# leslie-wang/hevcbitstream

Measured on AMD Instinct MI355X. Metric: Annex-B GB/s scanned + NAL units/s, 16 GiB synthetic stream, 1/2/4/8 MI355X, higher is better.
Workload: dtype u8

## Files before the change

hevcbitstream_amd/csrc/hbs_common.h:

```cpp
#ifndef HBS_COMMON_H
#define HBS_COMMON_H

#include <stdint.h>
#include <stddef.h>
#include "../../include/hevcbitstream_amd.h"

#if defined(__HIPCC__) && !defined(HBS_HOST_SIM)
#define HBS_HD __host__ __device__ __forceinline__
#define HBS_D  __device__ __forceinline__
#define HBS_M  __host__ __device__ __forceinline__
#else
#define HBS_HD static inline
#define HBS_D  static inline
#define HBS_M  inline
#endif

namespace hbs {

constexpr int kThreads         = 512;
constexpr int kWaves           = kThreads / 64;
constexpr int kBlockBytes      = 64;
constexpr int kBlocksPerThread = 2;
constexpr int kThreadBytes     = kBlockBytes * kBlocksPerThread;
constexpr int kTileBytes       = kThreads * kThreadBytes;
// ... 44 lines not shown
static_assert(sizeof(AheadCtl) == 64, "one line");
HBS_HD unsigned long long ahead_stamp_of(unsigned long long call) { return (call + 1ull) << 2; }

struct Carver {
    uint8_t* base;
    uint64_t at;
    template <class T> T* take(uint64_t bytes, uint64_t pack = 256)
    {
        T* const p = base ? reinterpret_cast<T*>(base + at) : nullptr;
        at += (bytes + pack - 1) / pack * pack;
        return p;
    }
};

constexpr uint64_t kOutCapMax = 1ull << 46;

constexpr uint32_t kDenseOneIn = 44;
constexpr int kExactFlagMin = 2;
constexpr uint32_t kDenseOneInIndexOnly = 9;
HBS_HD bool probe_says_dense(uint32_t chunks, uint32_t flagged, uint32_t one_in = kDenseOneIn) { return (uint64_t)flagged * one_in > (uint64_t)chunks; }
constexpr uint32_t kMidTwoIn = 13;
enum : int { kProbeSparse = 0, kProbeMid = 1, kProbeDense = 2 };
HBS_HD int probe_class(uint32_t chunks, uint32_t flagged, bool index_only)
{
    if (!probe_says_dense(chunks, flagged, index_only ? kDenseOneInIndexOnly : kDenseOneIn)) return kProbeSparse;
    return (uint64_t)flagged * kMidTwoIn > 2ull * (uint64_t)chunks ? kProbeDense : kProbeMid;
}
HBS_HD int probe_variant(uint32_t chunks, uint32_t flagged, bool index_only)
{
    const int c = probe_class(chunks, flagged, index_only);
    if (index_only) return c == kProbeSparse ? 5 : 2;
    return c == kProbeSparse ? 4 : c == kProbeMid ? 6 : 2;
}
enum : int { kGateNone = 0, kGateIfSparse = 1, kGateIfDense = 2, kGateIfSparseIdx = 3, kGateIfDenseIdx = 4, kGateIfMid = 5 };
#ifdef __HIPCC__
__device__ __forceinline__ int probe_class_dev(const RunHeader* __restrict__ hdr, bool index_only)
{
    const int lane = threadIdx.x & 63;
    uint32_t c = hdr->probe_slot[lane][0], f = hdr->probe_slot[lane][1];
#pragma unroll
    for (int d = 32; d >= 1; d >>= 1) { c += __shfl_xor(c, d, 64); f += __shfl_xor(f, d, 64); }
    return probe_class(c, f, index_only);
}
__device__ __forceinline__ bool gate_closed(int gate, const RunHeader* __restrict__ hdr)
{
    if (gate == kGateNone) return false;
    const bool idx = gate == kGateIfSparseIdx || gate == kGateIfDenseIdx;
    const int c = probe_class_dev(hdr, idx);
    if (idx) return (gate == kGateIfSparseIdx) != (c == kProbeSparse);
    const int want = gate == kGateIfSparse ? kProbeSparse : gate == kGateIfMid ? kProbeMid : kProbeDense;
    return c != want;
}
template <int kUnused = 0> __global__ void k_clear(uint8_t* __restrict__ p, uint64_t bytes)
{
    const uint64_t tid = (uint64_t)blockIdx.x * blockDim.x + threadIdx.x, step = (uint64_t)gridDim.x * blockDim.x;
    uint64_t head = (16u - (uint32_t)(reinterpret_cast<uintptr_t>(p) & 15u)) & 15u;
    if (head > bytes) head = bytes;
    const uint64_t whole = (bytes - head) / 16u;
    uint4* const q = reinterpret_cast<uint4*>(p + head);
    const uint4 z = make_uint4(0, 0, 0, 0);
    for (uint64_t i = tid; i < whole; i += step) q[i] = z;
    for (uint64_t i = tid; i < head; i += step) p[i] = 0;
    for (uint64_t i = head + 16u * whole + tid; i < bytes; i += step) p[i] = 0;
}
inline hipError_t clear_async(void* p, uint64_t bytes, hipStream_t st)
{
    if (!bytes) return hipSuccess;
    const uint64_t want = (bytes / 16u + 255u) / 256u;
    k_clear<0><<<dim3((unsigned)(want < 1 ? 1 : want > 1024 ? 1024 : want)), dim3(256), 0, st>>>(static_cast<uint8_t*>(p), bytes);
    return hipGetLastError();
}
inline hipError_t begin_launches(hipEvent_t ev_begin, hipStream_t st)
{
    return ev_begin ? hipEventRecord(ev_begin, st) : hipSuccess;
}
inline hipError_t end_launches(hipEvent_t ev_end, hipStream_t st)
{
    const hipError_t e = hipGetLastError();
    return e != hipSuccess || !ev_end ? e : hipEventRecord(ev_end, st);
}
#endif


HBS_HD uint32_t popc64(uint64_t v) { return (uint32_t)__builtin_popcountll(v); }
// ... 35 lines not shown
```

hevcbitstream_amd/csrc/hbs_scan.h:

```cpp
#ifndef HBS_SCAN_H
#define HBS_SCAN_H

#include <hip/hip_runtime_api.h>
#include <cassert>
#include "hbs_common.h"

namespace hbs {

struct ScanArgs {
    const uint8_t* stream;
    uint64_t n;
    hbs_nal_entry* index;
    uint64_t index_cap;
    uint8_t* rbsp;
    uint64_t rbsp_cap;
    unsigned long long* desc;
    RunHeader* hdr;
    uint8_t* tail;
    void* ws5;
    hbs_summary* summary;
    unsigned long long* ahead_cand;
    uint32_t* ahead_list;
    AheadCtl* ahead_ctl;
    void* ahead_tab;
    int grid_blocks;
    int grid_blocks4;
    int grid_blocks4r24;
    int first_static;
    int spare_wgs;
    hipEvent_t ev_begin, ev_end;
    int cus;
    int variant;
};

int scan_grid_blocks(int device, int* blocks_per_cu_out);
hipError_t launch_scan_extract(const ScanArgs& a, hipStream_t st);
inline bool scan_uses_index_only(uint64_t n, int variant, const void* rbsp)
{
    return rbsp == nullptr && (variant == 5 || (variant == 0 && n >= (1ull << 30)));
}
bool scan_takes_small_path(uint64_t n, uint64_t index_cap, int variant);

int scan4_grid_blocks(int device, int* blocks_per_cu_out);
int scan4_tile_bytes();
int scan4_tail_bytes();
void launch_scan_prologue(const ScanArgs& a, uint64_t desc_words, bool probe, int tail_tile_bytes , hipStream_t st);
void scan4_launch_kernel(const ScanArgs& a, uint64_t num_tiles, int gate, hipStream_t st);
int scan4r24_grid_blocks(int device, int* blocks_per_cu_out);
int scan4r24_tile_bytes();
void scan4r24_launch_kernel(const ScanArgs& a, uint64_t num_tiles, int gate, hipStream_t st);
uint64_t scan4_ahead_entry_bytes();
bool scan4_counts_ahead(uint64_t n);
void launch_scan_ahead4(const ScanArgs& a, uint64_t num_tiles, int gate, hipStream_t st);
inline uint64_t lay_scan_ahead(Carver& w, ScanArgs& a, uint64_t tiles)
{
    const uint64_t word = sizeof(unsigned long long), listed = sizeof(uint32_t), entry = scan4_ahead_entry_bytes() - word - listed;
    assert(entry == 64);
    a.ahead_ctl = w.take<AheadCtl>(sizeof(AheadCtl), 1);
    a.ahead_tab = w.take<void>(tiles * entry, 1);
    a.ahead_cand = w.take<unsigned long long>(tiles * word, 1);
    const uint64_t cleared = w.at;
    a.ahead_list = w.take<uint32_t>(tiles * listed, 1);
    return cleared;
}

uint64_t scan5_workspace_bytes(uint64_t stream_bytes);
struct Geo5 { int rows; int strided; uint64_t tiles, grid; };
Geo5 scan5_geometry(uint64_t n, uint64_t waves);
int scan5_tile_rows(uint64_t n, uint64_t waves);
void launch_scan_index5(const ScanArgs& a, int gate, hipStream_t st);

}
#endif
```

hevcbitstream_amd/csrc/hbs_scan.hip:

```cpp
#include <hip/hip_runtime.h>
#include "hbs_tile.h"
#include "hbs_scan.h"

namespace hbs {

#ifdef HBS_PHASE_TIMING
__device__ unsigned long long g_phase_cycles[1024][8];
#define HBS_T_DECL unsigned long long t_prev = __builtin_amdgcn_s_memtime(), t_acc[8] = {0,0,0,0,0,0,0,0};
#define HBS_T_MARK(i) { const unsigned long long t_now = __builtin_amdgcn_s_memtime(); t_acc[i] += t_now - t_prev; t_prev = t_now; }
#define HBS_T_COUNT(i, v) { t_acc[i] += (v); }
#define HBS_T_FLUSH if (threadIdx.x == 0 && blockIdx.x < 1024) { for (int i = 0; i < 8; ++i) g_phase_cycles[blockIdx.x][i] = t_acc[i]; }
__device__ int g_stop_after = 99;
#define HBS_T_STOP(i) if (g_stop_after == (i)) break;
#else
#define HBS_T_STOP(i)
#define HBS_T_DECL
#define HBS_T_MARK(i)
#define HBS_T_COUNT(i, v)
#define HBS_T_FLUSH
#endif

constexpr int kSlowCap = 256;

struct WaveSlot {
// ... 540 lines not shown
    if (per_cu < 1) per_cu = 1;
    if (blocks_per_cu_out) *blocks_per_cu_out = per_cu;
    return prop.multiProcessorCount * per_cu;
}

hipError_t launch_scan_extract(const ScanArgs& a, hipStream_t st)
{
    hipError_t e;
    const bool automatic = a.variant == 0;
    if (scan_takes_small_path(a.n, a.index_cap, a.variant)) {
        if (a.ev_begin) { e = hipEventRecord(a.ev_begin, st); if (e != hipSuccess) return e; }
        k_scan_small<<<1, dim3(kThreads), 0, st>>>(a.stream, a.n, a.index, a.index_cap, a.rbsp, a.rbsp_cap, a.desc, a.hdr, a.summary);
        if (a.ev_end) { e = hipEventRecord(a.ev_end, st); if (e != hipSuccess) return e; }
        return hipGetLastError();
    }
    const bool index_only = scan_uses_index_only(a.n, a.variant, a.rbsp);
    const int sparse_variant = ((a.variant == 5 && !index_only) || automatic) ? 4 : a.variant;
    const uint64_t tiles4 = (a.n + (uint64_t)scan4_tile_bytes() - 1) / (uint64_t)scan4_tile_bytes();
    const uint64_t tiles6 = (a.n + (uint64_t)scan4r24_tile_bytes() - 1) / (uint64_t)scan4r24_tile_bytes();
    const uint64_t tiles2 = (a.n + (uint64_t)kTileBytes - 1) / (uint64_t)kTileBytes;
    const uint64_t num_tiles = automatic ? tiles2 : sparse_variant == 4 ? tiles4 : sparse_variant == 6 ? tiles6 : tiles2;
    const int tail_tile = ((!index_only && sparse_variant == 4) || sparse_variant == 6 || automatic) ? scan4_tile_bytes() : 0;
    launch_scan_prologue(a, num_tiles * 2, automatic && a.n != 0, tail_tile, st);
    hipError_t first = hipSuccess;
    auto note = [&](hipError_t x) { if (first == hipSuccess && x != hipSuccess) first = x; };
    if (num_tiles) {
        uint64_t grid = (uint64_t)a.grid_blocks;
        if (grid > tiles2) grid = tiles2;
        if (a.ev_begin) note(hipEventRecord(a.ev_begin, st));
        if (index_only && !automatic) {
            launch_scan_index5(a, kGateNone, st);
        } else if (!automatic && sparse_variant == 4) {
            launch_scan_ahead4(a, tiles4, kGateNone, st);
            scan4_launch_kernel(a, tiles4, kGateNone, st);
        } else if (!automatic && sparse_variant == 6) {
            scan4r24_launch_kernel(a, tiles6, kGateNone, st);
        } else if (automatic) {
            if (index_only) launch_scan_index5(a, kGateIfSparseIdx, st);
            else { launch_scan_ahead4(a, tiles4, kGateIfSparse, st); scan4_launch_kernel(a, tiles4, kGateIfSparse, st); }
            if (!index_only) scan4r24_launch_kernel(a, tiles6, kGateIfMid, st);
            k_scan_extract<<<dim3((unsigned)grid), dim3(kThreads), 0, st>>>(
                a.stream, a.n, tiles2, a.index, a.index_cap, a.rbsp, a.rbsp_cap, a.desc, a.hdr, index_only ? kGateIfDenseIdx : kGateIfDense);
        } else {
            k_scan_extract<<<dim3((unsigned)grid), dim3(kThreads), 0, st>>>(
                a.stream, a.n, tiles2, a.index, a.index_cap, a.rbsp, a.rbsp_cap, a.desc, a.hdr, kGateNone);
        }
        if (a.ev_end) note(hipEventRecord(a.ev_end, st));
    }
    const uint64_t may = a.index_cap < a.n / 3 + 1 ? a.index_cap : a.n / 3 + 1;
    uint64_t fb = (may + 1023) / 1024;
    fb = fb < (uint64_t)kFinishBlocksMin ? (uint64_t)kFinishBlocksMin : fb > (uint64_t)kFinishBlocksMax ? (uint64_t)kFinishBlocksMax : fb;
    k_scan_finish<<<dim3((unsigned)fb), 256, 0, st>>>(a.stream, a.n, a.index, a.index_cap, a.rbsp, a.rbsp_cap, a.hdr, a.summary, a.ahead_ctl);
    note(hipGetLastError());
    return first;
}

}
```

hevcbitstream_amd/csrc/hbs_scan4.hip:

```cpp
#define HBS4_ROWS 48
#include "hbs_scan4_impl.h"
```

hevcbitstream_amd/csrc/hbs_scan4_impl.h:

```cpp
#include <hip/hip_runtime.h>
#ifndef HBS4_ROWS
#error "compile hbs_scan4.hip / hbs_scan4_r24.hip, which set HBS4_ROWS and include this file"
#endif
#include "hbs_wave.h"
#include "hbs_sparse.h"
#include "hbs_scan.h"
#include "hbs_elems.h"
#if HBS4_ROWS == 48
#include "hbs_scan4_rows48.h"
#define HBS4_KERNEL k_scan_extract4
#elif HBS4_ROWS == 24
#include "hbs_scan4_rows24.h"
#define HBS4_KERNEL k_scan_extract4_r24
#else
#error "no row lists for this HBS4_ROWS: scripts/set_rows4.py"
#endif
#define HBS4_MAIN (HBS4_ROWS == 48)

namespace hbs {
namespace {

#ifdef HBS_PHASE_TIMING
static __device__ unsigned long long g_phase_cycles4[1024][8];
#define HBS4_T_DECL unsigned long long t_prev = __builtin_amdgcn_s_memtime(), t_acc[8] = {0,0,0,0,0,0,0,0};
#define HBS4_T_MARK(i) { const unsigned long long t_now = __builtin_amdgcn_s_memtime(); t_acc[i] += t_now - t_prev; t_prev = t_now; }
#define HBS4_T_COUNT(i, v) { t_acc[i] += (v); }
#define HBS4_T_FLUSH if (threadIdx.x == 0 && blockIdx.x < 1024) { for (int i = 0; i < 8; ++i) g_phase_cycles4[blockIdx.x][i] = t_acc[i]; }
static __device__ uint32_t g_dbg4[4096];
constexpr unsigned kTl4Tiles = 1u << 17;
static __device__ unsigned long long g_tl4[kTl4Tiles][4];
static __device__ unsigned long long g_tlwho4[kTl4Tiles];
#define HBS4_TL(tile, k, bit) { if (threadIdx.x == 0 && (tile) < kTl4Tiles) { g_tl4[tile][k] = (wall_clock64() & ~1ull) | (unsigned long long)(bit); \
    if ((k) == 0) g_tlwho4[tile] = (unsigned long long)blockIdx.x | ((unsigned long long)(__builtin_amdgcn_s_getreg(63508) & 15u) << 28) | \
                                   ((unsigned long long)__builtin_amdgcn_s_getreg(63492) << 32); } }
static __device__ int g_fake_lb4 = 0;
#define HBS4_DBG(code) code
#else
#define HBS4_DBG(code)
#define HBS4_TL(tile, k, bit)
#define HBS4_T_DECL
#define HBS4_T_MARK(i)
#define HBS4_T_COUNT(i, v)
#define HBS4_T_FLUSH
#endif

constexpr int kWgPerCu = 2;
constexpr int kElemWaves = HBS4_ROWS == 48 ? 2 : 4;
constexpr int kCopyDepth = 3;
static_assert(k4Rows == HBS4_ROWS, "hbs_sparse.h takes the geometry from HBS4_ROWS");
constexpr int kParkRows = HBS4_PARK_ROWS;

struct RowRegs {
#define HBS_DECL(r) u32x4 q##r;
    HBS_ROWS(HBS_DECL)
#undef HBS_DECL
    uint32_t before;
    uint32_t before2;
    uint32_t after;
};

constexpr int kDepCap = 64;
constexpr uint32_t kDenseElems = HBS4_ROWS == 48 ? 512 : 1024;

struct Lds4 {
    uint32_t wave_tot[k4Waves];
    uint16_t wlist[k4Waves][kDenseElems];
    uint32_t seg[kDenseElems + 1];
    u32x4 rec[kDenseElems][3];
    Deposit dep[k4Waves][kDepCap];
    u32x4 park[kParkRows ? kElemWaves : 1][kParkRows ? kParkRows : 1][kParkRows ? 64 : 1];
    unsigned long long ex_kept, ex_nals;
    uint32_t ex_inside, ex_ok;
    uint32_t ticket;
    TileAgg wagg[k4Waves];
    TileAgg bagg[kDenseElems / k4ElemPass];
};


constexpr int kDenseAhead = 8;
static_assert(k4Rows % kDenseAhead == 0, "whole batches of rows");
template <class F>
__device__ __forceinline__ void dense_rows(const uint8_t* src, uint64_t wseg, int lane, F&& f)
// ... 171 lines not shown
        HBS4_TL(tile, 2, 0)
        __builtin_amdgcn_s_setprio(0);
        const uint32_t tile_kept = tagg.known + (ex.inside ? tagg.sig : 0u);
        const bool can = rbsp != nullptr && ex.kept + tile_kept <= rbsp_cap;
        if (lane == 0) {
            l.ex_kept = ex.kept; l.ex_nals = ex.nals; l.ex_inside = ex.inside;
            l.ex_ok = !ok ? 0u : (rbsp != nullptr && !can) ? 2u : 1u;
            if (ok && rbsp != nullptr && !can) atomicMax(&hdr->error, (uint32_t)(-HBS_E_CAPACITY));
            if (ok && last_tile) {
                const Prefix incl = fold(ex, tagg);
                hdr->final_kept = incl.kept; hdr->final_nals = incl.nals; hdr->final_inside = incl.inside;
            }
        }
    } else {
        __builtin_amdgcn_s_setprio(0);
    }
    __syncthreads();
    if (l.ex_ok == 0u) return false;
    Prefix excl;
    {
        Prefix ex;
        ex.kept = l.ex_kept; ex.nals = l.ex_nals; ex.inside = l.ex_inside;
        excl = prefix_uniform4(ex);
    }
    dense_emit(src, wseg, n, before, before2, after, chunk0, lane, before_me, excl, rbsp != nullptr && l.ex_ok == 1u, rbsp + excl.kept, tgt,
               &l.dep[wv][lane & (kDepCap - 1)].xpp);
    __syncthreads();
    if (tid == 0) l.ticket = ticket_base + atomicAdd(&hdr->ticket, 1u);
    __syncthreads();
    HBS4_TL(tile, 3, 0)
    return true;
}

}

#if HBS4_MAIN
__global__ __launch_bounds__(k4Threads)
void k_scan_ahead4(const uint8_t* __restrict__ stream, uint64_t n, uint64_t num_tiles, unsigned long long* __restrict__ cand,
                   const uint32_t* __restrict__ list, const AheadCtl* __restrict__ ctl,
                   AheadEntry* __restrict__ tab, const RunHeader* __restrict__ hdr, int gate)
{
    const uint32_t marked = ctl->listed;
    const unsigned long long stamp = ahead_stamp_of(ctl->call);
    if (blockIdx.x >= marked || gate_closed(gate, hdr)) return;
    __shared__ uint32_t rough[k4Waves];
    __shared__ TileAgg wagg[k4Waves];
    const int tid = threadIdx.x, lane = tid & 63;
    const int wv = __builtin_amdgcn_readfirstlane(tid >> 6);
    for (uint32_t i = blockIdx.x; i < marked; i += gridDim.x) {
        const uint64_t tile = list[i];
        if (tile + 1 >= num_tiles) continue;
        const uint64_t base = tile * (uint64_t)k4TileBytes;
        const uint64_t wseg = base + (uint64_t)(wv * k4WaveBytes);
        uint32_t mine = 0;
#pragma unroll 4
        for (int r = 0; r < k4Rows; ++r) {
            const Quad q = *reinterpret_cast<const Quad*>(stream + wseg + (uint64_t)r * k4RowBytes + (uint64_t)lane * 16u);
            mine += (uint32_t)__builtin_popcountll(__ballot(chunk_flag(0xFFFFFFFFu, q.x, q.y, q.z, q.w, 0xFFFFFFFFu)));
        }
        __syncthreads();
        if (lane == 0) rough[wv] = mine;
        __syncthreads();
        const bool walk = rough[0] + rough[1] + rough[2] + rough[3] >= kAheadRoughMin;
        if (!walk) continue;
        const uint32_t before = (wseg >= 4) ? stream_load4(stream + wseg - 4) : 0xFFFFFFFFu;
        const uint32_t before2 = (wseg >= 8) ? stream_load4(stream + wseg - 8) : 0xFFFFFFFFu;
        const uint32_t after = (wv != k4Waves - 1) ? stream_load4(stream + wseg + k4WaveBytes) : load_dword_guarded(stream, (int64_t)(wseg + k4WaveBytes), n);
        const TileAgg wa = dense_aggregate(stream, wseg, n, before, before2, after, (uint32_t)(64 * k4Rows * wv), lane);
        if (lane == 0) wagg[wv] = wa;
        __syncthreads();
        if (tid == 0) {
            AheadEntry e;
#pragma unroll
            for (int w = 0; w < k4Waves; ++w) e.w[w] = wagg[w];
            tab[tile] = e;
            cand[tile] = stamp | kAheadDone;
        }
    }
}

uint64_t scan4_ahead_entry_bytes() { return sizeof(AheadEntry) + sizeof(unsigned long long) + sizeof(uint32_t); }
bool scan4_counts_ahead(uint64_t n) { return n >= kAheadMinBytes; }

void launch_scan_ahead4(const ScanArgs& a, uint64_t num_tiles, int gate, hipStream_t st)
{
    if (!a.ahead_cand || !a.ahead_tab || num_tiles < 2) return;
    k_scan_ahead4<<<dim3(1024), dim3(k4Threads), 0, st>>>(a.stream, a.n, num_tiles, a.ahead_cand, a.ahead_list, a.ahead_ctl,
                                                         static_cast<AheadEntry*>(a.ahead_tab), a.hdr, gate);
}

#endif

__global__ __launch_bounds__(k4Threads, kWgPerCu)
void HBS4_KERNEL(const uint8_t* __restrict__ stream, uint64_t n, uint64_t num_tiles,
                 hbs_nal_entry* __restrict__ index, uint64_t index_cap,
                 uint8_t* __restrict__ rbsp, uint64_t rbsp_cap,
                 unsigned long long* __restrict__ desc, RunHeader* __restrict__ hdr, const uint8_t* __restrict__ tail, uint64_t tail_base,
                 int gate, int first_static)
{
    if (gate_closed(gate, hdr)) return;
    __shared__ Lds4 l;
    const int tid0 = threadIdx.x;
    const int wv = __builtin_amdgcn_readfirstlane(tid0 >> 6);
    EmitTarget tgt;
    tgt.index = index; tgt.index_cap = index_cap; tgt.hdr = hdr;
    const uint32_t ticket_base = first_static ? gridDim.x : 0u;
    if (tid0 == 0) l.ticket = first_static ? blockIdx.x : atomicAdd(&hdr->ticket, 1u);
    __syncthreads();
    HBS4_T_DECL

    uint32_t d_before = 0, d_before2 = 0, d_after = 0;
    uint64_t d_tile = 0;
    for (;;) {
    int pending = 0;
    for (;;) {
        int tid = launder_lane(tid0);
        int lane = tid & 63;
        const uint64_t tile = (uint64_t)(uint32_t)__builtin_amdgcn_readfirstlane((int)l.ticket);
        if (tile >= num_tiles) break;
        HBS4_TL(tile, 0, 0)
        const uint64_t base = tile * (uint64_t)k4TileBytes;
        const uint64_t tile_end = base + (uint64_t)k4TileBytes;
        const uint64_t wseg = base + (uint64_t)(wv * k4WaveBytes);
        const bool last_tile = tile == num_tiles - 1;
        const bool edge_tile = tile_end + 4 > n;

        const uint8_t* const src = last_tile
            ? reinterpret_cast<const uint8_t*>(reinterpret_cast<uintptr_t>(tail) + (uintptr_t)k4TailLead - (uintptr_t)tail_base) : stream;
        __builtin_amdgcn_s_setprio(3);
        RowRegs R;
        R.before = (wseg >= 4) ? stream_load4(src + wseg - 4) : 0xFFFFFFFFu;
        R.before2 = (wseg >= 8) ? stream_load4(src + wseg - 8) : 0xFFFFFFFFu;
        R.after = (last_tile || wv != k4Waves - 1) ? stream_load4(src + wseg + k4WaveBytes)
                                                   : load_dword_guarded(stream, (int64_t)(wseg + k4WaveBytes), n);
// ... 193 lines not shown
                    if (seg_inside(w) && cc < whole) \
                        arena_store16(out + (int64_t)seg_bias(w) + 16u * cc, R.q##r); \
                } else { \
                    const uint64_t f = HBS_ROW_FM(r); \
                    const uint32_t k = HBS_ROW_PRE(r) + lanes_below(f); \
                    if (!((f >> lane) & 1ull) && cc < whole) { \
                        const uint32_t w = l.seg[k]; \
                        if (seg_inside(w)) arena_store16(out + (int64_t)(seg_bias(w) + (int32_t)(16u * cc)), R.q##r); \
                    } \
                } \
                asm volatile("s_waitcnt vmcnt(%0)" :: "n"(kCopyDepth) : "memory"); }
            HBS_ROWS(HBS_COPY)
#undef HBS_COPY
        }
        if (tid == 0) l.ticket = ticket_base + atomicAdd(&hdr->ticket, 1u);
        __syncthreads();
        HBS4_T_MARK(5)
        HBS4_TL(tile, 3, 0)
#undef HBS_ROW_PRE
#undef HBS_ROW_FM
    }
    if (pending == 0) break;
    {
        const uint64_t base = d_tile * (uint64_t)k4TileBytes;
        const bool last_tile = d_tile == num_tiles - 1;
        const uint8_t* const src = last_tile
            ? reinterpret_cast<const uint8_t*>(reinterpret_cast<uintptr_t>(tail) + (uintptr_t)k4TailLead - (uintptr_t)tail_base) : stream;
        if (!dense_tile(l, src, base + (uint64_t)(wv * k4WaveBytes), n, d_before, d_before2, d_after, d_tile, last_tile, rbsp, rbsp_cap, desc, hdr, index, index_cap, ticket_base)) return;
    }
    }
    HBS4_T_FLUSH
}

#if HBS4_MAIN
#ifdef HBS_PHASE_TIMING
extern "C" int hbs_debug_fake_lb4(int on)
{
    return (int)hipMemcpyToSymbol(HIP_SYMBOL(g_fake_lb4), &on, sizeof(int));
}
extern "C" int hbs_debug_dump4(uint32_t* host_out )
{
    return (int)hipMemcpyFromSymbol(host_out, HIP_SYMBOL(g_dbg4), sizeof(uint32_t) * 4096);
}
extern "C" int hbs_debug_timeline4(unsigned long long* host_out , unsigned tiles)
{
    return (int)hipMemcpyFromSymbol(host_out, HIP_SYMBOL(g_tl4), sizeof(unsigned long long) * 4 * (tiles < kTl4Tiles ? tiles : kTl4Tiles));
}
extern "C" int hbs_debug_timeline_who4(unsigned long long* host_out , unsigned tiles)
{
    return (int)hipMemcpyFromSymbol(host_out, HIP_SYMBOL(g_tlwho4), sizeof(unsigned long long) * (tiles < kTl4Tiles ? tiles : kTl4Tiles));
}
extern "C" int hbs_debug_phase_cycles4(unsigned long long* host_out )
{
    return (int)hipMemcpyFromSymbol(host_out, HIP_SYMBOL(g_phase_cycles4), sizeof(unsigned long long) * 1024 * 8);
}
#endif

int scan4_tile_bytes() { return k4TileBytes; }
int scan4_tail_bytes() { return k4TailBytes; }

constexpr int kProbeBlocks = 64;
constexpr int kTailBlocks = 32;
constexpr int kClearBlocksMin = 32, kClearBlocksMax = 4096;

__global__ __launch_bounds__(256)
void k_scan_prologue(const uint8_t* __restrict__ stream, uint64_t n, RunHeader* __restrict__ hdr, uint8_t* __restrict__ tail,
                     unsigned long long* __restrict__ index_words, uint64_t n_index_words,
                     unsigned long long* __restrict__ desc, uint64_t n_desc_words, int do_probe, int tail_tile_bytes,
                     unsigned long long* __restrict__ ahead_cand, void* ahead_tab, uint32_t* __restrict__ ahead_list, AheadCtl* __restrict__ ahead_ctl,
                     int sample_blocks)
{
    if ((int)blockIdx.x >= (int)gridDim.x - sample_blocks) {
        const int lane = threadIdx.x & 63;
        const unsigned long long ahead_stamp = ahead_stamp_of(ahead_ctl->call);
        const uint64_t wave = ((uint64_t)(blockIdx.x - ((int)gridDim.x - sample_blocks)) * blockDim.x + threadIdx.x) >> 6;
        const uint64_t nwaves = ((uint64_t)sample_blocks * blockDim.x) >> 6;
        const uint64_t tiles = (n + (uint64_t)k4TileBytes - 1) / (uint64_t)k4TileBytes;
        static_assert(kAheadSample * 4096 == k4TileBytes && kAheadCoarse * 65536 == k4TileBytes, "a sample every 4 KiB, a coarse one every 64 KiB");
        auto hit = [&](uint64_t off) -> bool {
            if (off + 16 > n) return false;
            const Quad q = *reinterpret_cast<const Quad*>(stream + off);
            return chunk_flag(0xFFFFFFFFu, q.x, q.y, q.z, q.w, 0xFFFFFFFFu) && chunk_pattern_any_dev(0xFFFFFFFFu, q.x, q.y, q.z, q.w, 0xFFFFFFFFu);
        };
        for (uint64_t t0 = wave; t0 < tiles; t0 += nwaves * 16u) {
            const uint64_t ct = t0 + (uint64_t)(lane / kAheadCoarse) * nwaves;
            const bool ch = lane < 16 * kAheadCoarse && ct < tiles &&
                            hit(ct * (uint64_t)k4TileBytes + (uint64_t)(lane % kAheadCoarse) * 65536u + 32768u + 2048u);
            unsigned long long coarse = __ballot(ch);
            while (coarse != 0ull) {
                const int slot = __builtin_ctzll(coarse) / kAheadCoarse;
                const uint64_t t = t0 + (uint64_t)slot * nwaves;
// ... 65 lines not shown
        }
    } else {
        const uint64_t t0 = (uint64_t)(b - kProbeBlocks - kTailBlocks) * 256u + threadIdx.x;
        const uint64_t step = (uint64_t)((int)gridDim.x - sample_blocks - kProbeBlocks - kTailBlocks) * 256u;
        {
            const uint64_t head = (reinterpret_cast<uintptr_t>(index_words) & 8u) && n_index_words ? 1u : 0u;
            const uint64_t quads = (n_index_words - head) >> 1, rest = head + 2u * quads;
            u32x4* const q = reinterpret_cast<u32x4*>(index_words + head);
            for (uint64_t i = t0; i < quads; i += step) q[i] = u32x4{0u, 0u, 0u, 0u};
            if (t0 == 0 && head) index_words[0] = 0ull;
            if (t0 == 1 && rest < n_index_words) index_words[rest] = 0ull;
        }
        for (uint64_t i = t0; i < n_desc_words; i += step) desc[i] = 0ull;
    }
}

void launch_scan_prologue(const ScanArgs& a, uint64_t desc_words, bool probe, int tail_tile_bytes, hipStream_t st)
{
    const uint64_t index_words = a.index_cap * (sizeof(hbs_nal_entry) / 8);
    uint64_t clear_blocks = (index_words + desc_words) / (256u * 16u);
    if (clear_blocks < (uint64_t)kClearBlocksMin) clear_blocks = kClearBlocksMin;
    if (clear_blocks > (uint64_t)kClearBlocksMax) clear_blocks = kClearBlocksMax;
    unsigned sample_blocks = 0;
    if (a.ahead_cand && a.ahead_tab) {
        const uint64_t tiles = (a.n + (uint64_t)k4TileBytes - 1) / (uint64_t)k4TileBytes;
        const uint64_t want = (tiles + 63) / 64;
        sample_blocks = (unsigned)(want < 1 ? 1 : want > 512 ? 512 : want);
    }
    k_scan_prologue<<<dim3(kProbeBlocks + kTailBlocks + (unsigned)clear_blocks + sample_blocks), dim3(256), 0, st>>>(
        a.stream, a.n, a.hdr, a.tail, reinterpret_cast<unsigned long long*>(a.index), index_words,
        a.desc, desc_words, probe ? 1 : 0, tail_tile_bytes, a.ahead_cand, a.ahead_tab, a.ahead_list, a.ahead_ctl, (int)sample_blocks);
}

#endif
#if !HBS4_MAIN && defined(HBS_PHASE_TIMING)
extern "C" int hbs_debug_phase_cycles4_r24(unsigned long long* host_out )
{
    return (int)hipMemcpyFromSymbol(host_out, HIP_SYMBOL(g_phase_cycles4), sizeof(unsigned long long) * 1024 * 8);
}
#endif

#if HBS4_MAIN
#define HBS4_FN(name) scan4_##name
#else
#define HBS4_FN(name) scan4r24_##name
#endif
int HBS4_FN(grid_blocks)(int device, int* blocks_per_cu_out)
{
    hipDeviceProp_t prop;
    if (hipGetDeviceProperties(&prop, device) != hipSuccess) return -1;
    int per_cu = 0;
    if (hipOccupancyMaxActiveBlocksPerMultiprocessor(&per_cu, HBS4_KERNEL, k4Threads, 0) != hipSuccess) return -1;
    if (per_cu < 1) per_cu = 1;
    if (blocks_per_cu_out) *blocks_per_cu_out = per_cu;
    return prop.multiProcessorCount * per_cu;
}

#if !HBS4_MAIN
int scan4r24_tile_bytes() { return k4TileBytes; }
#endif

void HBS4_FN(launch_kernel)(const ScanArgs& a, uint64_t num_tiles, int gate, hipStream_t st)
{
    uint64_t grid = (uint64_t)(HBS4_MAIN ? a.grid_blocks4 : a.grid_blocks4r24);
    if (grid > num_tiles) grid = num_tiles;
    const uint64_t tail_tile = (uint64_t)scan4_tile_bytes();
    const uint64_t tail_base = a.n ? ((a.n - 1) / tail_tile) * tail_tile : 0;
    HBS4_KERNEL<<<dim3((unsigned)grid), dim3(k4Threads), 0, st>>>(
        a.stream, a.n, num_tiles, a.index, a.index_cap, a.rbsp, a.rbsp_cap, a.desc, a.hdr, a.tail, tail_base, gate, a.first_static);
}

}
```

hevcbitstream_amd/csrc/hbs_scan4_r24.hip:

```cpp
#define HBS4_ROWS 24
#include "hbs_scan4_impl.h"
```

hevcbitstream_amd/csrc/hbs_sparse.h:

```cpp
#ifndef HBS_SPARSE_H
#define HBS_SPARSE_H

#include "hbs_chunk.h"

namespace hbs {

#ifndef HBS4_ROWS
#define HBS4_ROWS 48
#endif
constexpr int k4Waves         = 4;
constexpr int k4Rows          = HBS4_ROWS;
constexpr int k4Threads       = 64 * k4Waves;
constexpr int k4RowBytes      = 1024;
constexpr int k4WaveBytes     = k4Rows * k4RowBytes;
constexpr int k4TileBytes     = k4Waves * k4WaveBytes;
constexpr int k4TileRows      = k4Waves * k4Rows;
constexpr int k4ChunksPerTile = k4TileBytes / kChunk;
constexpr int k4ElemPass      = 64;
constexpr int k4TailLead      = 16;
constexpr int k4TailBytes     = k4TailLead + k4TileBytes + 64;
static_assert(k4TileBytes >= kTileBytes, "the descriptor workspace is sized for kTileBytes tiles; larger tiles need less");
static_assert(k4ChunksPerTile <= 65536, "chunk numbers are kept in 16 bits");

HBS_HD uint32_t pk_min_u16(uint32_t a, uint32_t b)
{
#if defined(__HIP_DEVICE_COMPILE__)
    typedef unsigned short u16x2 __attribute__((ext_vector_type(2)));
    const u16x2 r = __builtin_elementwise_min(__builtin_bit_cast(u16x2, a), __builtin_bit_cast(u16x2, b));
    return __builtin_bit_cast(uint32_t, r);
#else
    const uint32_t lo = ((a & 0xFFFFu) < (b & 0xFFFFu)) ? (a & 0xFFFFu) : (b & 0xFFFFu);
    const uint32_t hi = ((a >> 16) < (b >> 16)) ? (a >> 16) : (b >> 16);
    return lo | (hi << 16);
#endif
}

HBS_HD bool chunk_flag(uint32_t xp, uint32_t x0, uint32_t x1, uint32_t x2, uint32_t x3, uint32_t xn)
{
    uint32_t m = pk_min_u16(xp | 0x0000FFFFu, x0);
    m = pk_min_u16(m, x1);
    m = pk_min_u16(m, x2);
    m = pk_min_u16(m, x3);
    m = pk_min_u16(m, alignbyte(x0, xp, 3));
    m = pk_min_u16(m, alignbyte(x1, x0, 3));
    m = pk_min_u16(m, alignbyte(x2, x1, 3));
    m = pk_min_u16(m, alignbyte(x3, x2, 3));
    m = pk_min_u16(m, alignbyte(xn, x3, 3));
    return (m & 0xFFFFu) == 0u || m < 0x10000u;
}

HBS_HD uint32_t span_bytes(uint64_t from, uint64_t to, uint64_t n)
{
    const uint64_t e = to < n ? to : n;
    return e > from ? (uint32_t)(e - from) : 0u;
}
// ... 170 lines not shown
```

Baseline: 2859.

## Merge sparse and mid scan kernels into one probe-dispatched auto kernel

In automatic mode the 48-row sparse kernel and the 24-row mid kernel, each launched and gated on the probe class, are replaced by a single kernel. It reads the probe class once and runs the matching geometry's tile loop from a shared LDS union. This removes one kernel launch and its early-exit blocks from the automatic path. In exchange, the combined kernel's LDS and register footprint is the larger of the two, which may reduce occupancy, and the grid is the smaller of the two grids.

```diff
diff --git a/hevcbitstream_amd/csrc/hbs_common.h b/hevcbitstream_amd/csrc/hbs_common.h
--- a/hevcbitstream_amd/csrc/hbs_common.h
+++ b/hevcbitstream_amd/csrc/hbs_common.h
@@ -100,7 +100,7 @@
     if (index_only) return c == kProbeSparse ? 5 : 2;
     return c == kProbeSparse ? 4 : c == kProbeMid ? 6 : 2;
 }
-enum : int { kGateNone = 0, kGateIfSparse = 1, kGateIfDense = 2, kGateIfSparseIdx = 3, kGateIfDenseIdx = 4, kGateIfMid = 5 };
+enum : int { kGateNone = 0, kGateIfSparse = 1, kGateIfDense = 2, kGateIfSparseIdx = 3, kGateIfDenseIdx = 4 };
 #ifdef __HIPCC__
 __device__ __forceinline__ int probe_class_dev(const RunHeader* __restrict__ hdr, bool index_only)
 {
@@ -116,8 +116,7 @@
     const bool idx = gate == kGateIfSparseIdx || gate == kGateIfDenseIdx;
     const int c = probe_class_dev(hdr, idx);
     if (idx) return (gate == kGateIfSparseIdx) != (c == kProbeSparse);
-    const int want = gate == kGateIfSparse ? kProbeSparse : gate == kGateIfMid ? kProbeMid : kProbeDense;
-    return c != want;
+    return c != (gate == kGateIfSparse ? kProbeSparse : kProbeDense);
 }
 template <int kUnused = 0> __global__ void k_clear(uint8_t* __restrict__ p, uint64_t bytes)
 {
diff --git a/hevcbitstream_amd/csrc/hbs_scan.h b/hevcbitstream_amd/csrc/hbs_scan.h
--- a/hevcbitstream_amd/csrc/hbs_scan.h
+++ b/hevcbitstream_amd/csrc/hbs_scan.h
@@ -45,10 +45,11 @@
 int scan4_tile_bytes();
 int scan4_tail_bytes();
 void launch_scan_prologue(const ScanArgs& a, uint64_t desc_words, bool probe, int tail_tile_bytes , hipStream_t st);
-void scan4_launch_kernel(const ScanArgs& a, uint64_t num_tiles, int gate, hipStream_t st);
+void scan4_launch_kernel(const ScanArgs& a, uint64_t num_tiles, hipStream_t st);
 int scan4r24_grid_blocks(int device, int* blocks_per_cu_out);
 int scan4r24_tile_bytes();
-void scan4r24_launch_kernel(const ScanArgs& a, uint64_t num_tiles, int gate, hipStream_t st);
+void scan4r24_launch_kernel(const ScanArgs& a, uint64_t num_tiles, hipStream_t st);
+void scan4_launch_auto(const ScanArgs& a, uint64_t num_tiles48, uint64_t num_tiles24, hipStream_t st);
 uint64_t scan4_ahead_entry_bytes();
 bool scan4_counts_ahead(uint64_t n);
 void launch_scan_ahead4(const ScanArgs& a, uint64_t num_tiles, int gate, hipStream_t st);
diff --git a/hevcbitstream_amd/csrc/hbs_scan.hip b/hevcbitstream_amd/csrc/hbs_scan.hip
--- a/hevcbitstream_amd/csrc/hbs_scan.hip
+++ b/hevcbitstream_amd/csrc/hbs_scan.hip
@@ -596,13 +596,12 @@
             launch_scan_index5(a, kGateNone, st);
         } else if (!automatic && sparse_variant == 4) {
             launch_scan_ahead4(a, tiles4, kGateNone, st);
-            scan4_launch_kernel(a, tiles4, kGateNone, st);
+            scan4_launch_kernel(a, tiles4, st);
         } else if (!automatic && sparse_variant == 6) {
-            scan4r24_launch_kernel(a, tiles6, kGateNone, st);
+            scan4r24_launch_kernel(a, tiles6, st);
         } else if (automatic) {
             if (index_only) launch_scan_index5(a, kGateIfSparseIdx, st);
-            else { launch_scan_ahead4(a, tiles4, kGateIfSparse, st); scan4_launch_kernel(a, tiles4, kGateIfSparse, st); }
-            if (!index_only) scan4r24_launch_kernel(a, tiles6, kGateIfMid, st);
+            else { launch_scan_ahead4(a, tiles4, kGateIfSparse, st); scan4_launch_auto(a, tiles4, tiles6, st); }
             k_scan_extract<<<dim3((unsigned)grid), dim3(kThreads), 0, st>>>(
                 a.stream, a.n, tiles2, a.index, a.index_cap, a.rbsp, a.rbsp_cap, a.desc, a.hdr, index_only ? kGateIfDenseIdx : kGateIfDense);
         } else {
diff --git a/hevcbitstream_amd/csrc/hbs_scan4.hip b/hevcbitstream_amd/csrc/hbs_scan4.hip
--- a/hevcbitstream_amd/csrc/hbs_scan4.hip
+++ b/hevcbitstream_amd/csrc/hbs_scan4.hip
@@ -1,2 +1,8 @@
 #define HBS4_ROWS 48
 #include "hbs_scan4_impl.h"
+#undef HBS4_ROWS
+#define HBS4_ROWS 24
+#include "hbs_scan4_impl.h"
+#undef HBS4_ROWS
+#define HBS4_ONCE
+#include "hbs_scan4_impl.h"
diff --git a/hevcbitstream_amd/csrc/hbs_scan4_impl.h b/hevcbitstream_amd/csrc/hbs_scan4_impl.h
--- a/hevcbitstream_amd/csrc/hbs_scan4_impl.h
+++ b/hevcbitstream_amd/csrc/hbs_scan4_impl.h
@@ -1,17 +1,20 @@
 #include <hip/hip_runtime.h>
-#ifndef HBS4_ROWS
-#error "compile hbs_scan4.hip / hbs_scan4_r24.hip, which set HBS4_ROWS and include this file"
-#endif
 #include "hbs_wave.h"
 #include "hbs_sparse.h"
 #include "hbs_scan.h"
 #include "hbs_elems.h"
+#ifndef HBS4_ONCE
+#ifndef HBS4_ROWS
+#error "compile hbs_scan4.hip, which sets HBS4_ROWS and includes this file once per geometry"
+#endif
 #if HBS4_ROWS == 48
 #include "hbs_scan4_rows48.h"
 #define HBS4_KERNEL k_scan_extract4
+#define HBS4_NS g48
 #elif HBS4_ROWS == 24
 #include "hbs_scan4_rows24.h"
 #define HBS4_KERNEL k_scan_extract4_r24
+#define HBS4_NS g24
 #else
 #error "no row lists for this HBS4_ROWS: scripts/set_rows4.py"
 #endif
@@ -19,6 +22,8 @@
 
 namespace hbs {
 namespace {
+namespace HBS4_NS {
+HBS4_GEOMETRY(HBS4_ROWS)
 
 #ifdef HBS_PHASE_TIMING
 static __device__ unsigned long long g_phase_cycles4[1024][8];
@@ -47,7 +52,7 @@
 constexpr int kWgPerCu = 2;
 constexpr int kElemWaves = HBS4_ROWS == 48 ? 2 : 4;
 constexpr int kCopyDepth = 3;
-static_assert(k4Rows == HBS4_ROWS, "hbs_sparse.h takes the geometry from HBS4_ROWS");
+static_assert(k4Rows == HBS4_ROWS, "this namespace's geometry (HBS4_GEOMETRY, hbs_sparse.h) is that of the row lists");
 constexpr int kParkRows = HBS4_PARK_ROWS;
 
 struct RowRegs {
@@ -285,74 +290,13 @@
     return true;
 }
 
-}
-
-#if HBS4_MAIN
-__global__ __launch_bounds__(k4Threads)
-void k_scan_ahead4(const uint8_t* __restrict__ stream, uint64_t n, uint64_t num_tiles, unsigned long long* __restrict__ cand,
-                   const uint32_t* __restrict__ list, const AheadCtl* __restrict__ ctl,
-                   AheadEntry* __restrict__ tab, const RunHeader* __restrict__ hdr, int gate)
-{
-    const uint32_t marked = ctl->listed;
-    const unsigned long long stamp = ahead_stamp_of(ctl->call);
-    if (blockIdx.x >= marked || gate_closed(gate, hdr)) return;
-    __shared__ uint32_t rough[k4Waves];
-    __shared__ TileAgg wagg[k4Waves];
-    const int tid = threadIdx.x, lane = tid & 63;
-    const int wv = __builtin_amdgcn_readfirstlane(tid >> 6);
-    for (uint32_t i = blockIdx.x; i < marked; i += gridDim.x) {
-        const uint64_t tile = list[i];
-        if (tile + 1 >= num_tiles) continue;
-        const uint64_t base = tile * (uint64_t)k4TileBytes;
-        const uint64_t wseg = base + (uint64_t)(wv * k4WaveBytes);
-        uint32_t mine = 0;
-#pragma unroll 4
-        for (int r = 0; r < k4Rows; ++r) {
-            const Quad q = *reinterpret_cast<const Quad*>(stream + wseg + (uint64_t)r * k4RowBytes + (uint64_t)lane * 16u);
-            mine += (uint32_t)__builtin_popcountll(__ballot(chunk_flag(0xFFFFFFFFu, q.x, q.y, q.z, q.w, 0xFFFFFFFFu)));
-        }
-        __syncthreads();
-        if (lane == 0) rough[wv] = mine;
-        __syncthreads();
-        const bool walk = rough[0] + rough[1] + rough[2] + rough[3] >= kAheadRoughMin;
-        if (!walk) continue;
-        const uint32_t before = (wseg >= 4) ? stream_load4(stream + wseg - 4) : 0xFFFFFFFFu;
-        const uint32_t before2 = (wseg >= 8) ? stream_load4(stream + wseg - 8) : 0xFFFFFFFFu;
-        const uint32_t after = (wv != k4Waves - 1) ? stream_load4(stream + wseg + k4WaveBytes) : load_dword_guarded(stream, (int64_t)(wseg + k4WaveBytes), n);
-        const TileAgg wa = dense_aggregate(stream, wseg, n, before, before2, after, (uint32_t)(64 * k4Rows * wv), lane);
-        if (lane == 0) wagg[wv] = wa;
-        __syncthreads();
-        if (tid == 0) {
-            AheadEntry e;
-#pragma unroll
-            for (int w = 0; w < k4Waves; ++w) e.w[w] = wagg[w];
-            tab[tile] = e;
-            cand[tile] = stamp | kAheadDone;
-        }
-    }
-}
-
-uint64_t scan4_ahead_entry_bytes() { return sizeof(AheadEntry) + sizeof(unsigned long long) + sizeof(uint32_t); }
-bool scan4_counts_ahead(uint64_t n) { return n >= kAheadMinBytes; }
-
-void launch_scan_ahead4(const ScanArgs& a, uint64_t num_tiles, int gate, hipStream_t st)
-{
-    if (!a.ahead_cand || !a.ahead_tab || num_tiles < 2) return;
-    k_scan_ahead4<<<dim3(1024), dim3(k4Threads), 0, st>>>(a.stream, a.n, num_tiles, a.ahead_cand, a.ahead_list, a.ahead_ctl,
-                                                         static_cast<AheadEntry*>(a.ahead_tab), a.hdr, gate);
-}
-
-#endif
-
-__global__ __launch_bounds__(k4Threads, kWgPerCu)
-void HBS4_KERNEL(const uint8_t* __restrict__ stream, uint64_t n, uint64_t num_tiles,
+__device__ __forceinline__
+void scan_tiles4(Lds4& l, const uint8_t* __restrict__ stream, uint64_t n, uint64_t num_tiles,
                  hbs_nal_entry* __restrict__ index, uint64_t index_cap,
                  uint8_t* __restrict__ rbsp, uint64_t rbsp_cap,
                  unsigned long long* __restrict__ desc, RunHeader* __restrict__ hdr, const uint8_t* __restrict__ tail, uint64_t tail_base,
-                 int gate, int first_static)
-{
-    if (gate_closed(gate, hdr)) return;
-    __shared__ Lds4 l;
+                 int first_static)
+{
     const int tid0 = threadIdx.x;
     const int wv = __builtin_amdgcn_readfirstlane(tid0 >> 6);
     EmitTarget tgt;
@@ -612,31 +556,179 @@
     HBS4_T_FLUSH
 }
 
+}
+}
+
+__global__ __launch_bounds__(k4Threads, HBS4_NS::kWgPerCu)
+void HBS4_KERNEL(const uint8_t* __restrict__ stream, uint64_t n, uint64_t num_tiles,
+                 hbs_nal_entry* __restrict__ index, uint64_t index_cap,
+                 uint8_t* __restrict__ rbsp, uint64_t rbsp_cap,
+                 unsigned long long* __restrict__ desc, RunHeader* __restrict__ hdr, const uint8_t* __restrict__ tail, uint64_t tail_base,
+                 int first_static)
+{
+    __shared__ HBS4_NS::Lds4 l;
+    HBS4_NS::scan_tiles4(l, stream, n, num_tiles, index, index_cap, rbsp, rbsp_cap, desc, hdr, tail, tail_base, first_static);
+}
+
+#ifdef HBS_PHASE_TIMING
 #if HBS4_MAIN
-#ifdef HBS_PHASE_TIMING
 extern "C" int hbs_debug_fake_lb4(int on)
 {
-    return (int)hipMemcpyToSymbol(HIP_SYMBOL(g_fake_lb4), &on, sizeof(int));
+    return (int)hipMemcpyToSymbol(HIP_SYMBOL(g48::g_fake_lb4), &on, sizeof(int));
 }
 extern "C" int hbs_debug_dump4(uint32_t* host_out )
 {
-    return (int)hipMemcpyFromSymbol(host_out, HIP_SYMBOL(g_dbg4), sizeof(uint32_t) * 4096);
+    return (int)hipMemcpyFromSymbol(host_out, HIP_SYMBOL(g48::g_dbg4), sizeof(uint32_t) * 4096);
 }
 extern "C" int hbs_debug_timeline4(unsigned long long* host_out , unsigned tiles)
 {
-    return (int)hipMemcpyFromSymbol(host_out, HIP_SYMBOL(g_tl4), sizeof(unsigned long long) * 4 * (tiles < kTl4Tiles ? tiles : kTl4Tiles));
+    return (int)hipMemcpyFromSymbol(host_out, HIP_SYMBOL(g48::g_tl4), sizeof(unsigned long long) * 4 * (tiles < g48::kTl4Tiles ? tiles : g48::kTl4Tiles));
 }
 extern "C" int hbs_debug_timeline_who4(unsigned long long* host_out , unsigned tiles)
 {
-    return (int)hipMemcpyFromSymbol(host_out, HIP_SYMBOL(g_tlwho4), sizeof(unsigned long long) * (tiles < kTl4Tiles ? tiles : kTl4Tiles));
+    return (int)hipMemcpyFromSymbol(host_out, HIP_SYMBOL(g48::g_tlwho4), sizeof(unsigned long long) * (tiles < g48::kTl4Tiles ? tiles : g48::kTl4Tiles));
 }
 extern "C" int hbs_debug_phase_cycles4(unsigned long long* host_out )
 {
-    return (int)hipMemcpyFromSymbol(host_out, HIP_SYMBOL(g_phase_cycles4), sizeof(unsigned long long) * 1024 * 8);
+    return (int)hipMemcpyFromSymbol(host_out, HIP_SYMBOL(g48::g_phase_cycles4), sizeof(unsigned long long) * 1024 * 8);
+}
+#else
+extern "C" int hbs_debug_phase_cycles4_r24(unsigned long long* host_out )
+{
+    return (int)hipMemcpyFromSymbol(host_out, HIP_SYMBOL(g24::g_phase_cycles4), sizeof(unsigned long long) * 1024 * 8);
 }
 #endif
-
-int scan4_tile_bytes() { return k4TileBytes; }
+#endif
+
+#if HBS4_MAIN
+#define HBS4_FN(name) scan4_##name
+#else
+#define HBS4_FN(name) scan4r24_##name
+#endif
+int HBS4_FN(grid_blocks)(int device, int* blocks_per_cu_out)
+{
+    hipDeviceProp_t prop;
+    if (hipGetDeviceProperties(&prop, device) != hipSuccess) return -1;
+    int per_cu = 0;
+    if (hipOccupancyMaxActiveBlocksPerMultiprocessor(&per_cu, HBS4_KERNEL, k4Threads, 0) != hipSuccess) return -1;
+    if (per_cu < 1) per_cu = 1;
+    if (blocks_per_cu_out) *blocks_per_cu_out = per_cu;
+    return prop.multiProcessorCount * per_cu;
+}
+
+int HBS4_FN(tile_bytes)() { return HBS4_NS::k4TileBytes; }
+
+void HBS4_FN(launch_kernel)(const ScanArgs& a, uint64_t num_tiles, hipStream_t st)
+{
+    uint64_t grid = (uint64_t)(HBS4_MAIN ? a.grid_blocks4 : a.grid_blocks4r24);
+    if (grid > num_tiles) grid = num_tiles;
+    const uint64_t tail_tile = (uint64_t)k4TileBytes;
+    const uint64_t tail_base = a.n ? ((a.n - 1) / tail_tile) * tail_tile : 0;
+    HBS4_KERNEL<<<dim3((unsigned)grid), dim3(k4Threads), 0, st>>>(
+        a.stream, a.n, num_tiles, a.index, a.index_cap, a.rbsp, a.rbsp_cap, a.desc, a.hdr, a.tail, tail_base, a.first_static);
+}
+
+}
+#undef HBS4_FN
+#undef HBS4_KERNEL
+#undef HBS4_NS
+#undef HBS4_MAIN
+#undef HBS_ROWS
+#undef HBS4_PARK_ROWS
+#undef HBS_PARKED
+#undef HBS_FLAG_PASS
+
+#else
+
+namespace hbs {
+namespace {
+using g48::AheadEntry; using g48::kAheadMinBytes; using g48::kAheadSample; using g48::kAheadMinHits; using g48::kAheadRoughMin;
+using g48::kAheadMarked; using g48::kAheadDone; using g48::kAheadCoarse;
+}
+
+union Lds4Both { g48::Lds4 r48; g24::Lds4 r24; };
+__global__ __launch_bounds__(k4Threads, g48::kWgPerCu)
+void k_scan_extract4_auto(const uint8_t* __restrict__ stream, uint64_t n, uint64_t num_tiles48, uint64_t num_tiles24,
+                          hbs_nal_entry* __restrict__ index, uint64_t index_cap,
+                          uint8_t* __restrict__ rbsp, uint64_t rbsp_cap,
+                          unsigned long long* __restrict__ desc, RunHeader* __restrict__ hdr, const uint8_t* __restrict__ tail, uint64_t tail_base,
+                          int first_static)
+{
+    __shared__ Lds4Both l;
+    const int c = __builtin_amdgcn_readfirstlane(probe_class_dev(hdr, false));
+    if (c == kProbeSparse) g48::scan_tiles4(l.r48, stream, n, num_tiles48, index, index_cap, rbsp, rbsp_cap, desc, hdr, tail, tail_base, first_static);
+    else if (c == kProbeMid) g24::scan_tiles4(l.r24, stream, n, num_tiles24, index, index_cap, rbsp, rbsp_cap, desc, hdr, tail, tail_base, first_static);
+}
+
+void scan4_launch_auto(const ScanArgs& a, uint64_t num_tiles48, uint64_t num_tiles24, hipStream_t st)
+{
+    static const int per_cu = [] {
+        int p = 0;
+        return hipOccupancyMaxActiveBlocksPerMultiprocessor(&p, k_scan_extract4_auto, k4Threads, 0) == hipSuccess && p >= 1 ? p : 1;
+    }();
+    uint64_t grid = (uint64_t)(a.grid_blocks4 < a.grid_blocks4r24 ? a.grid_blocks4 : a.grid_blocks4r24);
+    if (per_cu < g48::kWgPerCu) grid = (grid * (uint64_t)per_cu + g48::kWgPerCu - 1) / g48::kWgPerCu;
+    if (grid > num_tiles24) grid = num_tiles24;
+    const uint64_t tail_tile = (uint64_t)k4TileBytes;
+    const uint64_t tail_base = a.n ? ((a.n - 1) / tail_tile) * tail_tile : 0;
+    k_scan_extract4_auto<<<dim3((unsigned)grid), dim3(k4Threads), 0, st>>>(
+        a.stream, a.n, num_tiles48, num_tiles24, a.index, a.index_cap, a.rbsp, a.rbsp_cap, a.desc, a.hdr, a.tail, tail_base, a.first_static);
+}
+
+__global__ __launch_bounds__(k4Threads)
+void k_scan_ahead4(const uint8_t* __restrict__ stream, uint64_t n, uint64_t num_tiles, unsigned long long* __restrict__ cand,
+                   const uint32_t* __restrict__ list, const AheadCtl* __restrict__ ctl,
+                   AheadEntry* __restrict__ tab, const RunHeader* __restrict__ hdr, int gate)
+{
+    const uint32_t marked = ctl->listed;
+    const unsigned long long stamp = ahead_stamp_of(ctl->call);
+    if (blockIdx.x >= marked || gate_closed(gate, hdr)) return;
+    __shared__ uint32_t rough[k4Waves];
+    __shared__ TileAgg wagg[k4Waves];
+    const int tid = threadIdx.x, lane = tid & 63;
+    const int wv = __builtin_amdgcn_readfirstlane(tid >> 6);
+    for (uint32_t i = blockIdx.x; i < marked; i += gridDim.x) {
+        const uint64_t tile = list[i];
+        if (tile + 1 >= num_tiles) continue;
+        const uint64_t base = tile * (uint64_t)k4TileBytes;
+        const uint64_t wseg = base + (uint64_t)(wv * k4WaveBytes);
+        uint32_t mine = 0;
+#pragma unroll 4
+        for (int r = 0; r < k4Rows; ++r) {
+            const Quad q = *reinterpret_cast<const Quad*>(stream + wseg + (uint64_t)r * k4RowBytes + (uint64_t)lane * 16u);
+            mine += (uint32_t)__builtin_popcountll(__ballot(chunk_flag(0xFFFFFFFFu, q.x, q.y, q.z, q.w, 0xFFFFFFFFu)));
+        }
+        __syncthreads();
+        if (lane == 0) rough[wv] = mine;
+        __syncthreads();
+        const bool walk = rough[0] + rough[1] + rough[2] + rough[3] >= kAheadRoughMin;
+        if (!walk) continue;
+        const uint32_t before = (wseg >= 4) ? stream_load4(stream + wseg - 4) : 0xFFFFFFFFu;
+        const uint32_t before2 = (wseg >= 8) ? stream_load4(stream + wseg - 8) : 0xFFFFFFFFu;
+        const uint32_t after = (wv != k4Waves - 1) ? stream_load4(stream + wseg + k4WaveBytes) : load_dword_guarded(stream, (int64_t)(wseg + k4WaveBytes), n);
+        const TileAgg wa = g48::dense_aggregate(stream, wseg, n, before, before2, after, (uint32_t)(64 * k4Rows * wv), lane);
+        if (lane == 0) wagg[wv] = wa;
+        __syncthreads();
+        if (tid == 0) {
+            AheadEntry e;
+#pragma unroll
+            for (int w = 0; w < k4Waves; ++w) e.w[w] = wagg[w];
+            tab[tile] = e;
+            cand[tile] = stamp | kAheadDone;
+        }
+    }
+}
+
+uint64_t scan4_ahead_entry_bytes() { return sizeof(AheadEntry) + sizeof(unsigned long long) + sizeof(uint32_t); }
+bool scan4_counts_ahead(uint64_t n) { return n >= kAheadMinBytes; }
+
+void launch_scan_ahead4(const ScanArgs& a, uint64_t num_tiles, int gate, hipStream_t st)
+{
+    if (!a.ahead_cand || !a.ahead_tab || num_tiles < 2) return;
+    k_scan_ahead4<<<dim3(1024), dim3(k4Threads), 0, st>>>(a.stream, a.n, num_tiles, a.ahead_cand, a.ahead_list, a.ahead_ctl,
+                                                         static_cast<AheadEntry*>(a.ahead_tab), a.hdr, gate);
+}
+
 int scan4_tail_bytes() { return k4TailBytes; }
 
 constexpr int kProbeBlocks = 64;
@@ -768,42 +860,5 @@
         a.desc, desc_words, probe ? 1 : 0, tail_tile_bytes, a.ahead_cand, a.ahead_tab, a.ahead_list, a.ahead_ctl, (int)sample_blocks);
 }
 
+}
 #endif
-#if !HBS4_MAIN && defined(HBS_PHASE_TIMING)
-extern "C" int hbs_debug_phase_cycles4_r24(unsigned long long* host_out )
-{
-    return (int)hipMemcpyFromSymbol(host_out, HIP_SYMBOL(g_phase_cycles4), sizeof(unsigned long long) * 1024 * 8);
-}
-#endif
-
-#if HBS4_MAIN
-#define HBS4_FN(name) scan4_##name
-#else
-#define HBS4_FN(name) scan4r24_##name
-#endif
-int HBS4_FN(grid_blocks)(int device, int* blocks_per_cu_out)
-{
-    hipDeviceProp_t prop;
-    if (hipGetDeviceProperties(&prop, device) != hipSuccess) return -1;
-    int per_cu = 0;
-    if (hipOccupancyMaxActiveBlocksPerMultiprocessor(&per_cu, HBS4_KERNEL, k4Threads, 0) != hipSuccess) return -1;
-    if (per_cu < 1) per_cu = 1;
-    if (blocks_per_cu_out) *blocks_per_cu_out = per_cu;
-    return prop.multiProcessorCount * per_cu;
-}
-
-#if !HBS4_MAIN
-int scan4r24_tile_bytes() { return k4TileBytes; }
-#endif
-
-void HBS4_FN(launch_kernel)(const ScanArgs& a, uint64_t num_tiles, int gate, hipStream_t st)
-{
-    uint64_t grid = (uint64_t)(HBS4_MAIN ? a.grid_blocks4 : a.grid_blocks4r24);
-    if (grid > num_tiles) grid = num_tiles;
-    const uint64_t tail_tile = (uint64_t)scan4_tile_bytes();
-    const uint64_t tail_base = a.n ? ((a.n - 1) / tail_tile) * tail_tile : 0;
-    HBS4_KERNEL<<<dim3((unsigned)grid), dim3(k4Threads), 0, st>>>(
-        a.stream, a.n, num_tiles, a.index, a.index_cap, a.rbsp, a.rbsp_cap, a.desc, a.hdr, a.tail, tail_base, gate, a.first_static);
-}
-
-}
diff --git a/hevcbitstream_amd/csrc/hbs_scan4_r24.hip b/hevcbitstream_amd/csrc/hbs_scan4_r24.hip
--- a/hevcbitstream_amd/csrc/hbs_scan4_r24.hip
+++ /dev/null
@@ -1,2 +0,0 @@
-#define HBS4_ROWS 24
-#include "hbs_scan4_impl.h"
diff --git a/hevcbitstream_amd/csrc/hbs_sparse.h b/hevcbitstream_amd/csrc/hbs_sparse.h
--- a/hevcbitstream_amd/csrc/hbs_sparse.h
+++ b/hevcbitstream_amd/csrc/hbs_sparse.h
@@ -5,22 +5,21 @@
 
 namespace hbs {
 
-#ifndef HBS4_ROWS
-#define HBS4_ROWS 48
-#endif
 constexpr int k4Waves         = 4;
-constexpr int k4Rows          = HBS4_ROWS;
 constexpr int k4Threads       = 64 * k4Waves;
 constexpr int k4RowBytes      = 1024;
-constexpr int k4WaveBytes     = k4Rows * k4RowBytes;
-constexpr int k4TileBytes     = k4Waves * k4WaveBytes;
-constexpr int k4TileRows      = k4Waves * k4Rows;
-constexpr int k4ChunksPerTile = k4TileBytes / kChunk;
 constexpr int k4ElemPass      = 64;
 constexpr int k4TailLead      = 16;
-constexpr int k4TailBytes     = k4TailLead + k4TileBytes + 64;
-static_assert(k4TileBytes >= kTileBytes, "the descriptor workspace is sized for kTileBytes tiles; larger tiles need less");
-static_assert(k4ChunksPerTile <= 65536, "chunk numbers are kept in 16 bits");
+#define HBS4_GEOMETRY(ROWS) \
+    constexpr int k4Rows          = (ROWS); \
+    constexpr int k4WaveBytes     = k4Rows * k4RowBytes;          \
+    constexpr int k4TileBytes     = k4Waves * k4WaveBytes;        \
+    constexpr int k4TileRows      = k4Waves * k4Rows;             \
+    constexpr int k4ChunksPerTile = k4TileBytes / kChunk;         \
+    constexpr int k4TailBytes     = k4TailLead + k4TileBytes + 64; \
+    static_assert(k4TileBytes >= kTileBytes, "the descriptor workspace is sized for kTileBytes tiles; larger tiles need less"); \
+    static_assert(k4ChunksPerTile <= 65536, "chunk numbers are kept in 16 bits");
+HBS4_GEOMETRY(48)
 
 HBS_HD uint32_t pk_min_u16(uint32_t a, uint32_t b)
 {
```

Measured after the change: 2882, median of 2. About the same (+0.8%).
